# Avirup221/Multimodal-Hierarchical-CNN-for-Sun-Salutation-Pose-Classification

Measured on AMD Instinct MI355X. Metric: images/sec fwd+bwd QuadtreeCNN 224x224 bs256, higher is better.
Workload: dtype bf16; 1 GPU; QuadtreeCNN (ResNet-18 layer3, 2x2 split, 47-feat fusion) train step fwd+bwd+Adam, all parameters trainable; Adam(lr 1e-4, wd 1e-4) by the package's FusedAdam (csrc/pack.hip); global_batch=256, per_gpu_batch=256, image=3x224x224, num_classes=12, parallelism=dp1

## Files before the change

include/qtcnn.h:

```cpp
#ifndef QTCNN_H_
#define QTCNN_H_

#include <stddef.h>
#include <stdint.h>

#ifdef __cplusplus
extern "C" {
#endif

typedef enum qt_status {
  QT_OK = 0,
  QT_ERR_INVALID_ARG = -1,
  QT_ERR_LAUNCH = -2,
  QT_ERR_UNSUPPORTED = -3
} qt_status;

typedef enum qt_dtype { QT_F32 = 0, QT_BF16 = 1 } qt_dtype;

int qt_version(void);
const char* qt_last_error(void);

enum { QT_CONV_FWD = 0, QT_CONV_DGRAD = 1 };

typedef struct qt_conv_desc {
// ... 7 lines not shown
  int kh, kw, stride, pad;
  long long src_img_stride;
  int src_row_stride;
  int src_pix_stride;
  int quad;
  int relu;
  int dst_sub, dst_h, dst_w, dst_off_h, dst_off_w;
  int dst_merge;
  int dst_merge_res0;
  int kt, frames;
  int dst_merge_extra;
} qt_conv_desc;

typedef struct qt_conv_io {
  const void* src;
  const void* weight;
  void* dst;
  const float* scale;
  const float* shift;
  const void* residual;
  const void* relu_mask;
  float* stats_partial;
  struct {
    const void* y;
    const float* mean;
    const float* invstd;
    float* partial;
  } bwd_bn[2];
  const unsigned char* relu_mask_bits;
  const void* extra_src;
} qt_conv_io;

void qt_set_patch_conv(int mode);
void qt_set_pt_conv(int mode);
void qt_set_pt_conv_max_workgroups(int n);
void qt_set_stem_conv(int mode);
int qt_conv2d_stats_rows(const qt_conv_desc* desc);
typedef struct qt_conv_s2_desc {
  int dtype;
  int batch;
  int in_h, in_w;
  int c_in, c_out;
  int relu_conv, relu_down;
} qt_conv_s2_desc;
typedef struct qt_conv_s2_io {
  const void* src;
  const void* w_conv;
  const void* w_down;
  void* y_conv;
  void* y_down;
  const float* scale_conv;
  const float* shift_conv;
  const float* scale_down;
  const float* shift_down;
  float* stats_conv;
  float* stats_down;
} qt_conv_s2_io;
int qt_conv_s2_pair_supported(const qt_conv_s2_desc* desc);
int qt_conv_s2_pair_stats_rows(const qt_conv_s2_desc* desc);
int qt_conv_s2_pair(const qt_conv_s2_desc* desc, const qt_conv_s2_io* io, void* stream);
void qt_set_conv_s2(int mode);
void qt_set_conv_s2_max_workgroups(int n);

int qt_conv2d_igemm(const qt_conv_desc* desc, const qt_conv_io* io, void* stream);

int qt_conv2d_wgrad(const qt_conv_desc* desc, const void* dy, const void* x, float* dw, void* stream);
// ... 228 lines not shown
```

multimodal-hierarchical-cnn-for-sun-salutation-pose-classification_amd/csrc/conv_patch.hip:

```cpp
#include <stdlib.h>

#include <type_traits>

#include "qt_common.h"

namespace {

struct PatchArgs {
  const void* src;
  const void* wgt;
  void* dst;
  const float* scale;
  const float* shift;
  const void* residual;
  const void* relu_mask;
  const unsigned char* relu_mask_bits;
  float* stats_partial;
  const void* bn_y[2];
  const float* bn_mean[2];
  const float* bn_invstd[2];
  float* bn_partial[2];
  int B, H, W, C, N;
  int PW, PP;
  long long Q;
  int flip;
  int relu;
  int gridM, gridN;
  FastDiv div_pp, div_pw;
};

constexpr int kRowBytes = 128;
constexpr int BM = 256;
constexpr int NT = 512;

constexpr int L1_PW = 58, L1_RING = 640, L1_MIRROR = 48, L1_WBYTES = 9 * 64 * kRowBytes;
constexpr int L1_RBYTES = (L1_RING + L1_MIRROR) * kRowBytes;
constexpr int L1_RED = 0;
constexpr int L1_LDS = L1_WBYTES + L1_RBYTES;
static_assert(L1_LDS <= 160 * 1024 && 8 * 2 * 4 * 4 * 3 * 4 <= L1_WBYTES, "layer1 ring kernel LDS");

__device__ uint4 l1_store_sink[NT];

template <bool FLIP, bool OPS>
__global__ __launch_bounds__(NT) void conv_l1_ring_kernel(PatchArgs p) {
  using T = bf16_t;
  extern __shared__ __attribute__((aligned(16))) unsigned char smem[];
  const T* __restrict__ src = static_cast<const T*>(p.src);
  const T* __restrict__ wgt = static_cast<const T*>(p.wgt);
  const int tid = threadIdx.x, lane = tid & 63;
  const int wave = __builtin_amdgcn_readfirstlane(tid >> 6);
  const int wm = wave & 3, wn = wave >> 2;
  const int frow = lane & 15, fk = lane >> 4;
  const int rbase = tid >> 3, chunk = (tid & 7) ^ (rbase & 7);
  const unsigned smem_base = lds_addr_of(smem);
  const T* zero_src = reinterpret_cast<const T*>(qt_zero_page);

  const int ntiles = p.gridM, G = gridDim.x, b = blockIdx.x;
  const int t0 = (int)((long long)b * ntiles / G), t1 = (int)((long long)(b + 1) * ntiles / G);
  const int nt = t1 - t0;
  if (nt <= 0) return;
  const long long qstart = (long long)t0 * BM - (L1_PW + 1);

  auto dma_ring = [&](int ub) {
    const long long q = qstart + ub + rbase;
    const T* g = zero_src;
    if (q >= 0 && q < p.Q) {
      const unsigned uq = (unsigned)q;
      const unsigned img = fdiv(uq, p.div_pp);
      const unsigned rem = uq - img * (unsigned)p.PP;
      const unsigned hp = fdiv(rem, p.div_pw);
      const unsigned wp = rem - hp * (unsigned)L1_PW;
      if (hp >= 1 && hp <= 56u && wp >= 1 && wp <= 56u)
        g = src + (((long long)img * 56 + (hp - 1)) * 56 + (wp - 1)) * 64 + chunk * 8;
    }
    const int rrow = __builtin_amdgcn_readfirstlane(ub % L1_RING);
    glds16(g, smem_base + L1_WBYTES + (rrow + wave * 8) * kRowBytes);
    if (rrow == 0 && wave < L1_MIRROR / 8)
// ... 6 lines not shown
    const int x = rbase & 15, ii = (rbase >> 4) & 1;
    const int chan = (rbase & 32) + 8 * (x >> 2) + 4 * ii + (x & 3);
    glds16(wgt + ((long long)chan * 9 + t) * 64 + chunk * 8, smem_base + (t * 64 + wave * 8) * kRowBytes);
  }
#pragma unroll
  for (int i = 0; i < 6; ++i) dma_ring(i * 64);

  float sc[2][4], sh[2][4], mu0[2][4], is0[2][4], mu1[2][4], is1[2][4];
  const bool bwd_stats = p.bn_y[0] != nullptr;
#pragma unroll
  for (int i = 0; i < 2; ++i)
#pragma unroll
    for (int r = 0; r < 4; ++r) {
      const int n = wn * 32 + fk * 8 + i * 4 + r;
      sc[i][r] = p.scale ? p.scale[n] : 1.f;
      sh[i][r] = p.shift ? p.shift[n] : 0.f;
      mu0[i][r] = bwd_stats ? p.bn_mean[0][n] : 0.f;
      is0[i][r] = bwd_stats ? p.bn_invstd[0][n] : 0.f;
      mu1[i][r] = p.bn_y[1] ? p.bn_mean[1][n] : 0.f;
      is1[i][r] = p.bn_y[1] ? p.bn_invstd[1][n] : 0.f;
    }
  float s1[2][4], s2[2][4], s3[2][4];
#pragma unroll
  for (int i = 0; i < 2; ++i)
#pragma unroll
    for (int r = 0; r < 4; ++r) s1[i][r] = s2[i][r] = s3[i][r] = 0.f;
  T* __restrict__ dst = static_cast<T*>(p.dst);
  const T* __restrict__ res = static_cast<const T*>(p.residual);
  const T* __restrict__ msk = static_cast<const T*>(p.relu_mask);
  const unsigned char* __restrict__ mbits = p.relu_mask_bits;
  const unsigned char* ring = smem + L1_WBYTES;
  const int w_lane = (wn * 32 + frow) * kRowBytes + ((fk ^ (frow & 7)) << 4);

  int base = 0;
  for (int k = 0; k < nt; ++k) {
    if (k == 0)
      asm volatile("s_waitcnt vmcnt(0) lgkmcnt(0)\n\ts_barrier" ::: "memory");
    else
      asm volatile("s_waitcnt vmcnt(4) lgkmcnt(0)\n\ts_barrier" ::: "memory");
    if (k + 1 < nt) {
#pragma unroll
      for (int i = 0; i < 4; ++i) dma_ring(256 * k + 384 + i * 64);
    }
    auto out_row = [&](int j) -> int {
      const long long q = (long long)(t0 + k) * BM + wm * 64 + j * 16 + frow;
      if (q >= p.Q) return -1;
      const unsigned uq = (unsigned)q;
      const unsigned img = fdiv(uq, p.div_pp);
      const unsigned rem = uq - img * (unsigned)p.PP;
      const unsigned hp = fdiv(rem, p.div_pw);
      const unsigned wp = rem - hp * (unsigned)L1_PW;
      return (hp >= 1 && hp <= 56u && wp >= 1 && wp <= 56u) ? (int)((img * 56 + (hp - 1)) * 56 + (wp - 1)) : -1;
    };
    int prow[4] = {-1, -1, -1, -1};
    uint4 pre_res[4], pre_msk[4], pre_y0[4], pre_y1[4];
    if constexpr (OPS) {
#pragma unroll
      for (int j = 0; j < 4; ++j) {
        prow[j] = out_row(j);
        pre_res[j] = pre_msk[j] = pre_y0[j] = pre_y1[j] = make_uint4(0u, 0u, 0u, 0u);
        if (prow[j] >= 0) {
          const long long off = (long long)prow[j] * 64 + wn * 32 + fk * 8;
          if (res) pre_res[j] = *reinterpret_cast<const uint4*>(res + off);
          if (msk) pre_msk[j] = *reinterpret_cast<const uint4*>(msk + off);
          if (mbits) pre_msk[j].x = mbits[off >> 3];
          if (bwd_stats) pre_y0[j] = *reinterpret_cast<const uint4*>(static_cast<const T*>(p.bn_y[0]) + off);
          if (p.bn_y[1]) pre_y1[j] = *reinterpret_cast<const uint4*>(static_cast<const T*>(p.bn_y[1]) + off);
        }
      }
    }
    f32x4 acc[2][4];
#pragma unroll
    for (int i = 0; i < 2; ++i)
#pragma unroll
      for (int j = 0; j < 4; ++j) acc[i][j] = (f32x4){0.f, 0.f, 0.f, 0.f};
    const int lane_row = base + wm * 64 + frow;
    uint4 fwp[2][2], fap[2][4];
    auto read_group = [&](int g, uint4 (&fw)[2], uint4 (&fa)[4]) {
      constexpr int kPW = L1_PW;
      const int t = g >> 1, kk = g & 1;
      const int kh = t / 3, kw = t % 3;
      const int shift = FLIP ? (2 - kh) * kPW + (2 - kw) : kh * kPW + kw;
      int rr0 = lane_row + shift;
      rr0 = rr0 >= L1_RING ? rr0 - L1_RING : rr0;
      const int a0 = rr0 * kRowBytes + ((fk ^ ((frow + shift) & 7)) << 4);
#pragma unroll
      for (int i = 0; i < 2; ++i)
        fw[i] = *reinterpret_cast<const uint4*>(smem + (w_lane ^ (kk << 6)) + (t * 64 + i * 16) * kRowBytes);
#pragma unroll
      for (int j = 0; j < 4; ++j)
        fa[j] = *reinterpret_cast<const uint4*>(ring + (a0 ^ (kk << 6)) + j * (16 * kRowBytes));
    };
    read_group(0, fwp[0], fap[0]);
#pragma unroll
    for (int g = 0; g < 18; ++g) {
      if (g + 1 < 18) read_group(g + 1, fwp[(g + 1) & 1], fap[(g + 1) & 1]);
      __builtin_amdgcn_sched_barrier(0);
      __builtin_amdgcn_s_setprio(1);
#pragma unroll
      for (int i = 0; i < 2; ++i)
#pragma unroll
        for (int j = 0; j < 4; ++j) QtMma<T>::run(acc[i][j], fwp[g & 1][i], fap[g & 1][j]);
      __builtin_amdgcn_s_setprio(0);
      __builtin_amdgcn_sched_barrier(0);
    }
    base += BM;
    if (base >= L1_RING) base -= L1_RING;

    auto bf4 = [](unsigned lo, unsigned hi, float (&f)[4]) {
      f[0] = __uint_as_float(lo << 16); f[1] = __uint_as_float(lo & 0xffff0000u);
      f[2] = __uint_as_float(hi << 16); f[3] = __uint_as_float(hi & 0xffff0000u);
    };
#pragma unroll
    for (int j = 0; j < 4; ++j) {
      if constexpr (!OPS) prow[j] = out_row(j);
      const bool live = prow[j] >= 0;
      const float lm = live ? 1.f : 0.f;
      const long long off = (long long)(live ? prow[j] : 0) * 64 + wn * 32 + fk * 8;
      bf16x8 o;
#pragma unroll
      for (int i = 0; i < 2; ++i) {
        float v[4] = {acc[i][j][0], acc[i][j][1], acc[i][j][2], acc[i][j][3]};
        if (p.stats_partial != nullptr && !bwd_stats) {
#pragma unroll
          for (int r = 0; r < 4; ++r) {
// ... 69 lines not shown
        for (int r = 0; r < 4; ++r) {
          float* d = red + ((((wave * 2 + i) * 4 + fk) * 4 + r) * 3);
          d[0] = s1[i][r];
          d[1] = s2[i][r];
          d[2] = s3[i][r];
        }
    }
    __syncthreads();
    if (tid < 64) {
      const int n = tid, wn_ = n >> 5, fk_ = (n >> 3) & 3, i = (n >> 2) & 1, r = n & 3;
      float a = 0.f, bb = 0.f, c = 0.f;
      for (int w4 = 0; w4 < 4; ++w4) {
        const float* d = red + (((((wn_ * 4 + w4) * 2 + i) * 4 + fk_) * 4 + r) * 3);
        a += d[0];
        bb += d[1];
        c += d[2];
      }
      float* o0 = bwd_stats ? p.bn_partial[0] : p.stats_partial;
      o0[((long long)b * 2 + 0) * 64 + n] = a;
      o0[((long long)b * 2 + 1) * 64 + n] = bb;
      if (bwd_stats && p.bn_y[1]) {
        p.bn_partial[1][((long long)b * 2 + 0) * 64 + n] = a;
        p.bn_partial[1][((long long)b * 2 + 1) * 64 + n] = c;
      }
    }
  }
}

inline int l1_ring_grid(long long Q) {
  const int ntiles = qt_cdiv(Q, BM);
  return ntiles < 256 ? ntiles : 256;
}

template <bool FLIP, bool OPS>
int launch_l1_ring(PatchArgs a, hipStream_t stream) {
  auto kern = conv_l1_ring_kernel<FLIP, OPS>;
  static std::atomic<unsigned long long> lds_limit_set{0};
  if (int rc = qt_raise_lds_limit(reinterpret_cast<const void*>(kern), L1_LDS, lds_limit_set)) return rc;
  a.gridM = qt_cdiv(a.Q, BM);
  a.gridN = 1;
  hipLaunchKernelGGL(kern, dim3(l1_ring_grid(a.Q)), dim3(NT), L1_LDS, stream, a);
  QT_CHECK_LAUNCH();
  return QT_OK;
}

}



static int g_patch_enabled = -1;
extern "C" void qt_set_patch_conv(int mode) { g_patch_enabled = mode < 0 ? 2 : (mode > 2 ? 2 : mode); }

static bool l1_ring_shape(const qt_conv_desc* d);

bool qt_patch_eligible(const qt_conv_desc* d) {
  if (g_patch_enabled < 0) {
    const char* v = getenv("QTCNN_PATCH_CONV");
    g_patch_enabled = v ? atoi(v) : 2;
  }
  if (!g_patch_enabled) return false;
  return l1_ring_shape(d) && d->kh == 3 && d->kw == 3 && d->stride == 1 && d->pad == 1 && !d->quad && !d->dst_sub &&
         d->in_h == d->out_h && d->in_w == d->out_w && d->in_h == d->in_w && d->src_pix_stride == d->k_per_tap &&
         d->src_row_stride == d->in_w * d->k_per_tap &&
         d->src_img_stride == (long long)d->in_h * d->in_w * d->k_per_tap &&
         (long long)d->batch * (d->in_h + 2) * (d->in_w + 2) < (1ll << 31);
}

static bool l1_ring_shape(const qt_conv_desc* d) {
  return d->dtype == QT_BF16 && d->in_w == 56 && d->k_per_tap == 64 && d->n_out == 64;
}

int qt_patch_stats_rows(const qt_conv_desc* d) {
  const long long Q = (long long)d->batch * (d->in_h + 2) * (d->in_w + 2);
  return l1_ring_grid(Q);
}

int qt_patch_launch(const qt_conv_desc* d, const qt_conv_io* io, void* stream) {
  PatchArgs a;
  a.src = io->src; a.wgt = io->weight; a.dst = io->dst;
  a.scale = io->scale; a.shift = io->shift; a.residual = io->residual; a.relu_mask = io->relu_mask;
  a.relu_mask_bits = io->relu_mask_bits;
  a.stats_partial = io->stats_partial;
  for (int k = 0; k < 2; ++k) {
    a.bn_y[k] = io->bwd_bn[k].y; a.bn_mean[k] = io->bwd_bn[k].mean; a.bn_invstd[k] = io->bwd_bn[k].invstd;
    a.bn_partial[k] = io->bwd_bn[k].partial;
  }
  a.B = d->batch; a.H = d->in_h; a.W = d->in_w; a.C = d->k_per_tap; a.N = d->n_out;
  a.PW = a.W + 2; a.PP = (a.H + 2) * a.PW;
  a.Q = (long long)a.B * a.PP;
  a.flip = d->mode == QT_CONV_DGRAD;
  a.relu = d->relu;
  a.div_pp = make_fastdiv((unsigned)a.PP);
  a.div_pw = make_fastdiv((unsigned)a.PW);
  a.gridM = a.gridN = 0;
  hipStream_t s = static_cast<hipStream_t>(stream);
  const bool ops = a.residual || a.relu_mask || a.relu_mask_bits || a.bn_y[0];
  if (a.flip) return ops ? launch_l1_ring<true, true>(a, s) : launch_l1_ring<true, false>(a, s);
  return ops ? launch_l1_ring<false, true>(a, s) : launch_l1_ring<false, false>(a, s);
}
```

multimodal-hierarchical-cnn-for-sun-salutation-pose-classification_amd/csrc/conv_wgrad_s2.hip:

```cpp
#include <stdlib.h>

#include "qt_common.h"

int qt_wgrad_partial_sum_launch(const float* part, float* dw, size_t filt, int nsplit, int KC, int layout, hipStream_t stream);

namespace {

constexpr int T = 64;
constexpr int CH = 32;

struct WS2Args {
  const bf16_t* dy;
  const bf16_t* x;
  float* part;
  unsigned x_is2, dy_is2;
  int x_rs, x_ps;
  int N, KC, OH, OW, PW, PP, B;
  int total, pps, nsplit, tiles, tilesC;
  int HL;
  unsigned xrb, bufb, tab;
  unsigned x_bytes, dy_bytes;
  FastDiv div_pp, div_pw;
  int tap_plane[9], tap_shift[9];
};

__device__ __forceinline__ QT_LDS_AS s16x4* lds_tr_ptr(unsigned lds_byte) { return (QT_LDS_AS s16x4*)(size_t)lds_byte; }

template <int NPL, int NTAP, int NB, int NU>
__global__ __launch_bounds__(512) void conv_wgrad_s2_kernel(WS2Args a) {
  extern __shared__ __attribute__((aligned(16))) unsigned char smem[];
  if (lds_addr_of(smem) != 0) return;

  const int tid = threadIdx.x, lane = tid & 63;
  const int wave = __builtin_amdgcn_readfirstlane(tid >> 6);
  const int group = wave >> 2, wq = wave & 3;

  int split, tile;
  if ((a.nsplit & 7) == 0) {
    const int xcd = blockIdx.x & 7, slot = blockIdx.x >> 3;
    split = (slot / a.tiles) * 8 + xcd;
    tile = slot % a.tiles;
  } else {
    split = blockIdx.x % a.nsplit;
    tile = blockIdx.x / a.nsplit;
  }
  const int tc = tile % a.tilesC, tn = tile / a.tilesC;
  const int n0 = tn * 64, c0 = tc * 64;
  const int p0 = split * a.pps;
  if (p0 >= a.total) return;
  const int pend = min(a.total, p0 + a.pps);
  const int ntiles = (pend - p0 + T - 1) / T;

  const int tabn = a.PP + 8;
  {
    unsigned* tx = reinterpret_cast<unsigned*>(smem + a.tab);
    unsigned* ty = tx + tabn;
    for (int r = tid; r < tabn; r += 512) {
      const int rr = r >= a.PP ? r - a.PP : r;
      const int ph = (int)fdiv((unsigned)rr, a.div_pw), pw = rr - ph * a.PW;
      const bool ok = ph >= 1 && pw >= 1;
      const unsigned nx = r >= a.PP ? a.x_is2 : 0u, ny = r >= a.PP ? a.dy_is2 : 0u;
      tx[r] = ok ? (unsigned)(2 * (ph - 1) * a.x_rs + 2 * (pw - 1) * a.x_ps) * 2u + nx : kOob;
      ty[r] = ok ? (unsigned)(((ph - 1) * a.OW + (pw - 1)) * a.N) * 2u + ny : kOob;
    }
  }

  const i32x4 rx = make_rsrc(a.x, a.x_bytes), ry = make_rsrc(a.dy, a.dy_bytes);
  const int drow = lane >> 3, dslot = lane & 7;
  const int dkey = (drow >> 1) & 3;
  const unsigned lane_c = (unsigned)((((dslot >> 1) ^ dkey) << 1) | (dslot & 1)) * 16u;
  const unsigned tab_x = a.tab + (unsigned)drow * 4u, tab_y = tab_x + (unsigned)tabn * 4u;
  const int xu = (T + a.HL) >> 3;
  const int xunits = NPL * xu;
  auto sgpr = [](unsigned v) -> unsigned { return (unsigned)__builtin_amdgcn_readfirstlane((int)v); };
  auto split_pos = [&](int pos, unsigned& img1, unsigned& rem) {
    const unsigned g = (unsigned)(pos + a.PP);
    img1 = fdiv(g, a.div_pp);
    rem = g - img1 * (unsigned)a.PP;
  };
  const unsigned spare = a.tab + 2u * (unsigned)tabn * 4u;
  auto dma_tile = [&](int k, unsigned bufbase) {
    const int q0 = p0 + k * T;
#pragma unroll
    for (int j = 0; j < NU - 1; ++j) {
      const int u = wave + 8 * j;
      const bool live = u < xunits;
      const int uc = live ? u : 0;
      const int pl = NPL == 1 ? 0 : uc / xu, uu = NPL == 1 ? uc : uc - pl * xu;
      unsigned img1, rem;
      split_pos(q0 - a.HL + 8 * uu, img1, rem);
      const unsigned plane_off = (unsigned)((pl >> 1) * a.x_rs + (pl & 1) * a.x_ps) * 2u;
      const unsigned base = sgpr((img1 - 1u) * a.x_is2 + (unsigned)c0 * 2u + plane_off);
      const unsigned tv = *reinterpret_cast<const unsigned*>(smem + tab_x + sgpr(rem) * 4u);
      i32x4 r_ = rx;
      r_.z = (int)sgpr(live ? a.x_bytes : 0u);
      blds16(r_, tv + base + lane_c, 0u, sgpr(live ? bufbase + (unsigned)pl * a.xrb + (unsigned)uu * 1024u : spare));
    }
    {
      unsigned img1, rem;
      split_pos(q0 + 8 * wave, img1, rem);
      const unsigned base = sgpr((img1 - 1u) * a.dy_is2 + (unsigned)n0 * 2u);
      const unsigned tv = *reinterpret_cast<const unsigned*>(smem + tab_y + sgpr(rem) * 4u);
      blds16(ry, tv + base + lane_c, 0u, sgpr(bufbase + (unsigned)NPL * a.xrb + (unsigned)wave * 1024u));
    }
  };

  const int li = lane & 15, lg = lane >> 4;
  const int qq = li >> 2, pp = li & 3;
  const int lrow = 4 * lg + qq;
  unsigned a_base[4], b_base[NTAP];
#pragma unroll
  for (int i = 0; i < 4; ++i)
    a_base[i] = (unsigned)NPL * a.xrb + (unsigned)(group * CH + lrow) * 128u + ((unsigned)(i ^ ((lrow >> 1) & 3)) << 5) + pp * 8;
#pragma unroll
  for (int t = 0; t < NTAP; ++t) {
    const int r = a.HL + a.tap_shift[t] + group * CH + lrow;
    b_base[t] = (unsigned)a.tap_plane[t] * a.xrb + (unsigned)r * 128u + ((unsigned)(wq ^ ((r >> 1) & 3)) << 5) + pp * 8;
  }
  auto frag = [&](unsigned addr) -> uint4 {
    s16x4 lo = __builtin_amdgcn_ds_read_tr16_b64_v4i16(lds_tr_ptr(addr));
    s16x4 hi = __builtin_amdgcn_ds_read_tr16_b64_v4i16(lds_tr_ptr(addr + 2048));
    uint2 l2 = __builtin_bit_cast(uint2, lo), h2 = __builtin_bit_cast(uint2, hi);
    return make_uint4(l2.x, l2.y, h2.x, h2.y);
  };

  f32x4 acc[4][NTAP];
#pragma unroll
  for (int i = 0; i < 4; ++i)
#pragma unroll
    for (int t = 0; t < NTAP; ++t) acc[i][t] = (f32x4){0.f, 0.f, 0.f, 0.f};

  asm volatile("s_waitcnt lgkmcnt(0)\n\ts_barrier" ::: "memory");
#pragma unroll
  for (int t = 0; t < NB - 1; ++t) dma_tile(t, (unsigned)t * a.bufb);
  asm volatile("s_waitcnt vmcnt(%0) lgkmcnt(0)\n\ts_barrier" ::"n"(NU * (NB - 2)) : "memory");

  unsigned wbuf = (unsigned)(NB - 1) * a.bufb;
  int rbuf = 0;
  for (int k = 0; k < ntiles; ++k) {
    dma_tile(k + NB - 1, wbuf);
    wbuf = wbuf + a.bufb == (unsigned)NB * a.bufb ? 0u : wbuf + a.bufb;
    uint4 fa[4], fb[3];
#pragma unroll
    for (int i = 0; i < 4; ++i) fa[i] = frag(a_base[i]);
    fb[0] = frag(b_base[0]);
    if (NTAP > 1) fb[1] = frag(b_base[NTAP > 1 ? 1 : 0]);
#pragma unroll
    for (int t = 0; t < NTAP; ++t) {
      if (t + 2 < NTAP) fb[(t + 2) % 3] = frag(b_base[t + 2 < NTAP ? t + 2 : 0]);
      __builtin_amdgcn_s_setprio(1);
#pragma unroll
      for (int i = 0; i < 4; ++i)
        acc[i][t] = __builtin_amdgcn_mfma_f32_16x16x32_bf16(__builtin_bit_cast(bf16x8, fa[i]),
                                                            __builtin_bit_cast(bf16x8, fb[t % 3]), acc[i][t], 0, 0, 0);
      __builtin_amdgcn_s_setprio(0);
    }
    {
      rbuf = rbuf + 1 == NB ? 0 : rbuf + 1;
      const unsigned delta = rbuf == 0 ? 0u - (unsigned)(NB - 1) * a.bufb : a.bufb;
#pragma unroll
      for (int i = 0; i < 4; ++i) {
        a_base[i] += delta;
        asm volatile("" : "+v"(a_base[i]));
      }
#pragma unroll
      for (int t = 0; t < NTAP; ++t) {
        b_base[t] += delta;
        asm volatile("" : "+v"(b_base[t]));
      }
    }
    asm volatile("s_waitcnt vmcnt(%0) lgkmcnt(0)\n\ts_barrier" ::"n"(NU * (NB - 2)) : "memory");
  }
  asm volatile("s_waitcnt vmcnt(0)" ::: "memory");
  __syncthreads();

  {
    f32x4* xch = reinterpret_cast<f32x4*>(smem) + (wq * 2 * NTAP) * 64 + lane;
    if (group == 1) {
#pragma unroll
      for (int i = 0; i < 2; ++i)
#pragma unroll
        for (int t = 0; t < NTAP; ++t) xch[(i * NTAP + t) * 64] = acc[i][t];
    }
    __syncthreads();
    if (group == 0) {
#pragma unroll
      for (int i = 0; i < 2; ++i)
#pragma unroll
        for (int t = 0; t < NTAP; ++t) acc[i][t] += xch[(i * NTAP + t) * 64];
    }
    __syncthreads();
    if (group == 0) {
#pragma unroll
      for (int i = 0; i < 2; ++i)
#pragma unroll
        for (int t = 0; t < NTAP; ++t) xch[(i * NTAP + t) * 64] = acc[2 + i][t];
    }
    __syncthreads();
    if (group == 1) {
#pragma unroll
      for (int i = 0; i < 2; ++i)
// ... 33 lines not shown

int s2_buffers() {
  static int v = -1;
  if (v < 0) {
    const char* e = getenv("QTCNN_S2_BUFFERS");
    v = e ? atoi(e) : 3;
  }
  return v;
}

void split_ranges(int total, int tiles, int* pps_out, int* nsplit_out) {
  int nsplit = 256 / tiles;
  if (nsplit < 1) nsplit = 1;
  int pps = qt_cdiv(total, nsplit);
  pps = qt_cdiv(pps, T) * T;
  *pps_out = pps;
  *nsplit_out = qt_cdiv(total, pps);
}

}

extern "C" void qt_set_wgrad_s2(int on) { g_wgrad_s2 = on < 0 ? 1 : on; }

bool qt_wgrad_s2_eligible(const qt_conv_desc* d) {
  if (!s2_enabled() || d->dtype != QT_BF16 || d->stride != 2 || d->quad || d->kt > 1) return false;
  const bool k3 = d->kh == 3 && d->kw == 3 && d->pad == 1, k1 = d->kh == 1 && d->kw == 1 && d->pad == 0;
  if (!k3 && !k1) return false;
  if ((d->in_h & 1) || (d->in_w & 1) || d->out_h * 2 != d->in_h || d->out_w * 2 != d->in_w) return false;
  if (d->n_out % 64 || d->k_per_tap % 64) return false;
  if (d->out_w < 4 || d->out_w > 120 || d->out_h < 4) return false;
  if ((long long)d->batch * d->src_img_stride * 2 >= (1ll << 30)) return false;
  if ((long long)d->batch * d->out_h * d->out_w * d->n_out * 2 >= (1ll << 30)) return false;
  if ((long long)d->batch * (d->out_h + 1) * (d->out_w + 1) >= (1ll << 30)) return false;
  const int PW = d->out_w + 1, HL = (PW + 1 + 7) / 8 * 8;
  const unsigned npl = k3 ? 4u : 1u;
  const unsigned lds = 2u * ((npl * (unsigned)(T + HL) + (unsigned)T) * 128u) + 2u * (unsigned)((d->out_h + 1) * PW + 8) * 4u + 1024u;
  const int nu = qt_cdiv((int)npl * ((T + HL) / 8), 8) + 1;
  if (k3 ? (nu != 6 && nu != 7) : (nu != 2 && nu != 3)) return false;
  return lds <= 160u * 1024u && HL <= (d->out_h + 1) * PW;
}

size_t qt_wgrad_s2_workspace_bytes(const qt_conv_desc* d) {
  if (!qt_wgrad_s2_eligible(d)) return 0;
  const int total = d->batch * (d->out_h + 1) * (d->out_w + 1);
  int pps, nsplit;
  split_ranges(total, (d->n_out / 64) * (d->k_per_tap / 64), &pps, &nsplit);
  return (size_t)nsplit * d->n_out * d->kh * d->kw * d->k_per_tap * 4;
}

int qt_wgrad_s2_launch(const qt_conv_desc* d, const void* dy, const void* x, float* grad_oihw, void* workspace,
                       size_t workspace_bytes, void* stream) {
  const bool k3 = d->kh == 3;
  WS2Args a;
  a.dy = static_cast<const bf16_t*>(dy);
  a.x = static_cast<const bf16_t*>(x);
  a.part = static_cast<float*>(workspace);
  a.N = d->n_out; a.KC = d->k_per_tap; a.OH = d->out_h; a.OW = d->out_w; a.B = d->batch;
  a.PW = a.OW + 1; a.PP = a.PW * (a.OH + 1);
  a.x_rs = d->src_row_stride; a.x_ps = d->src_pix_stride;
  a.x_is2 = (unsigned)(d->src_img_stride * 2);
  a.dy_is2 = (unsigned)((long long)a.OH * a.OW * a.N * 2);
  a.x_bytes = (unsigned)((long long)a.B * d->src_img_stride * 2);
  a.dy_bytes = (unsigned)((long long)a.B * a.OH * a.OW * a.N * 2);
  a.total = a.B * a.PP;
  a.HL = (a.PW + 1 + 7) / 8 * 8;
  a.div_pp = make_fastdiv((unsigned)a.PP);
  a.div_pw = make_fastdiv((unsigned)a.PW);
  a.tilesC = a.KC / 64;
  a.tiles = (a.N / 64) * a.tilesC;
  int real_split;
  split_ranges(a.total, a.tiles, &a.pps, &real_split);
  a.nsplit = real_split;
  if (a.nsplit >= 6 && (a.nsplit & 7)) a.nsplit = qt_cdiv(a.nsplit, 8) * 8;
  const int ntap = k3 ? 9 : 1, npl = k3 ? 4 : 1;
  const size_t filt = (size_t)a.N * ntap * a.KC;
  if (!workspace || workspace_bytes < (size_t)real_split * filt * 4) {
    qt_set_error("qt_conv2d_wgrad_oihw: workspace of %zu bytes needed", (size_t)real_split * filt * 4);
    return QT_ERR_INVALID_ARG;
  }
  a.xrb = (unsigned)(T + a.HL) * 128u;
  a.bufb = (unsigned)npl * a.xrb + (unsigned)T * 128u;
  const unsigned tab_bytes = 2u * (unsigned)(a.PP + 8) * 4u + 1024u;
  const int nb = (3u * a.bufb + tab_bytes <= 160u * 1024u && s2_buffers() >= 3) ? 3 : 2;
  a.tab = (unsigned)nb * a.bufb;
  const int nu = qt_cdiv(npl * ((T + a.HL) / 8), 8) + 1;
  for (int t = 0; t < 9; ++t) {
    const int kh = k3 ? t / 3 : 1, kw = k3 ? t % 3 : 1;
    a.tap_plane[t] = k3 ? ((kh != 1) * 2 + (kw != 1)) : 0;
    a.tap_shift[t] = -((kh == 0) * a.PW + (kw == 0));
  }
  const unsigned lds = a.tab + tab_bytes;
  if ((size_t)2 * a.bufb < (size_t)4 * 2 * ntap * 64 * 16) {
    qt_set_error("qt_conv2d_wgrad_oihw: map too small for the stride-2 kernel");
    return QT_ERR_UNSUPPORTED;
  }
  hipStream_t s = static_cast<hipStream_t>(stream);
#define QT_S2_LAUNCH(NPL_, NTAP_, NB_, NU_)                                                                     \
  {                                                                                                             \
    auto kern = conv_wgrad_s2_kernel<NPL_, NTAP_, NB_, NU_>;                                                    \
    static std::atomic<unsigned long long> set_{0};                                                             \
    if (int rc = qt_raise_lds_limit(reinterpret_cast<const void*>(kern), 160 * 1024, set_)) return rc;          \
    hipLaunchKernelGGL(kern, dim3(a.tiles * a.nsplit), dim3(512), lds, s, a);                                   \
    launched = true;                                                                                            \
  }
  bool launched = false;
  if (k3 && nb == 3 && nu == 6) QT_S2_LAUNCH(4, 9, 3, 6)
  else if (k3 && nb == 3 && nu == 7) QT_S2_LAUNCH(4, 9, 3, 7)
  else if (k3 && nu == 6) QT_S2_LAUNCH(4, 9, 2, 6)
  else if (k3 && nu == 7) QT_S2_LAUNCH(4, 9, 2, 7)
  else if (!k3 && nb == 3 && nu == 3) QT_S2_LAUNCH(1, 1, 3, 3)
  else if (!k3 && nb == 3 && nu == 2) QT_S2_LAUNCH(1, 1, 3, 2)
  else if (!k3 && nu == 3) QT_S2_LAUNCH(1, 1, 2, 3)
  else if (!k3 && nu == 2) QT_S2_LAUNCH(1, 1, 2, 2)
#undef QT_S2_LAUNCH
  if (!launched) {
    qt_set_error("qt_conv2d_wgrad_oihw: stride-2 kernel: no instantiation for this map width");
    return QT_ERR_UNSUPPORTED;
  }
  QT_CHECK_LAUNCH();
  return qt_wgrad_partial_sum_launch(a.part, grad_oihw, filt, real_split, a.KC, k3 ? 1 : 2, s);
}
```

Before: 46020 images/s.

## Overlap layer1 ring conv epilogue with next tile's MFMA loop

Adds a pipelined variant of the layer1 ring conv kernel for the no-memory-operand case. It double-buffers the accumulators, and the previous tile's epilogue (address calc, stats accumulation, affine/relu, bf16 pack, global store) is interleaved into the next tile's 18 MFMA groups using sched_group_barrier hints. The ring DMA prefetches are also spread across the first groups instead of issued up front. This aims to hide epilogue latency behind matrix work, at the cost of doubled accumulator registers and a spill risk. It is enabled by default and can be turned off with QTCNN_L1_PIPE=0.

```diff
diff --git a/include/qtcnn.h b/include/qtcnn.h
--- a/include/qtcnn.h
+++ b/include/qtcnn.h
@@ -63,6 +63,7 @@
 } qt_conv_io;
 
 void qt_set_patch_conv(int mode);
+void qt_set_l1_pipe(int mode);
 void qt_set_pt_conv(int mode);
 void qt_set_pt_conv_max_workgroups(int n);
 void qt_set_stem_conv(int mode);
diff --git a/multimodal-hierarchical-cnn-for-sun-salutation-pose-classification_amd/csrc/conv_patch.hip b/multimodal-hierarchical-cnn-for-sun-salutation-pose-classification_amd/csrc/conv_patch.hip
--- a/multimodal-hierarchical-cnn-for-sun-salutation-pose-classification_amd/csrc/conv_patch.hip
+++ b/multimodal-hierarchical-cnn-for-sun-salutation-pose-classification_amd/csrc/conv_patch.hip
@@ -41,8 +41,9 @@
 
 __device__ uint4 l1_store_sink[NT];
 
-template <bool FLIP, bool OPS>
+template <bool FLIP, bool OPS, int PIPE>
 __global__ __launch_bounds__(NT) void conv_l1_ring_kernel(PatchArgs p) {
+  static_assert(PIPE == 0 || !OPS, "the pipelined epilogue has no memory operands");
   using T = bf16_t;
   extern __shared__ __attribute__((aligned(16))) unsigned char smem[];
   const T* __restrict__ src = static_cast<const T*>(p.src);
@@ -115,7 +116,154 @@
   const unsigned char* ring = smem + L1_WBYTES;
   const int w_lane = (wn * 32 + frow) * kRowBytes + ((fk ^ (frow & 7)) << 4);
 
+  auto read_group_at = [&](int lane_row, int g, uint4 (&fw)[2], uint4 (&fa)[4]) {
+    constexpr int kPW = L1_PW;
+    const int t = g >> 1, kk = g & 1;
+    const int kh = t / 3, kw = t % 3;
+    const int shift = FLIP ? (2 - kh) * kPW + (2 - kw) : kh * kPW + kw;
+    int rr0 = lane_row + shift;
+    rr0 = rr0 >= L1_RING ? rr0 - L1_RING : rr0;
+    const int a0 = rr0 * kRowBytes + ((fk ^ ((frow + shift) & 7)) << 4);
+#pragma unroll
+    for (int i = 0; i < 2; ++i)
+      fw[i] = *reinterpret_cast<const uint4*>(smem + (w_lane ^ (kk << 6)) + (t * 64 + i * 16) * kRowBytes);
+#pragma unroll
+    for (int j = 0; j < 4; ++j)
+      fa[j] = *reinterpret_cast<const uint4*>(ring + (a0 ^ (kk << 6)) + j * (16 * kRowBytes));
+  };
+  auto out_row_at = [&](int tile, int j) -> int {
+    const long long q = (long long)tile * BM + wm * 64 + j * 16 + frow;
+    if (q >= p.Q) return -1;
+    const unsigned uq = (unsigned)q;
+    const unsigned img = fdiv(uq, p.div_pp);
+    const unsigned rem = uq - img * (unsigned)p.PP;
+    const unsigned hp = fdiv(rem, p.div_pw);
+    const unsigned wp = rem - hp * (unsigned)L1_PW;
+    return (hp >= 1 && hp <= 56u && wp >= 1 && wp <= 56u) ? (int)((img * 56 + (hp - 1)) * 56 + (wp - 1)) : -1;
+  };
+
   int base = 0;
+  if constexpr (PIPE != 0) {
+    if constexpr (PIPE == 2) {
+#pragma unroll
+      for (int i = 0; i < 2; ++i)
+#pragma unroll
+        for (int r = 0; r < 4; ++r) asm volatile("" ::"v"(sc[i][r]), "v"(sh[i][r]));
+    }
+    float lm = 0.f;
+    bf16x8* outp = nullptr;
+    bf16x8 o;
+    auto part_addr = [&](int tile, int j) {
+      int fr = frow;
+      asm volatile("" : "+v"(fr));
+      const long long q = (long long)tile * BM + wm * 64 + j * 16 + fr;
+      const unsigned uq = (unsigned)q;
+      const unsigned img = fdiv(uq, p.div_pp);
+      const unsigned rem = uq - img * (unsigned)p.PP;
+      const unsigned hp = fdiv(rem, p.div_pw);
+      const unsigned wp = rem - hp * (unsigned)L1_PW;
+      const bool live = q < p.Q && hp >= 1 && hp <= 56u && wp >= 1 && wp <= 56u;
+      const int row = (int)((img * 56 + (hp - 1)) * 56 + (wp - 1));
+      lm = live ? 1.f : 0.f;
+      const long long off = (long long)(live ? row : 0) * 64 + wn * 32 + fk * 8;
+      outp = live ? reinterpret_cast<bf16x8*>(dst + off) : reinterpret_cast<bf16x8*>(&l1_store_sink[tid]);
+      asm volatile("" ::"v"(lm), "v"(outp));
+    };
+    auto part_half = [&](const f32x4 (&prv)[2][4], int j, int i) {
+      float v[4] = {prv[i][j][0], prv[i][j][1], prv[i][j][2], prv[i][j][3]};
+      asm volatile("" : "+v"(v[0]), "+v"(v[1]), "+v"(v[2]), "+v"(v[3]));
+#pragma unroll
+      for (int r = 0; r < 4; ++r) {
+        s1[i][r] += lm * v[r];
+        s2[i][r] += lm * v[r] * v[r];
+      }
+      if constexpr (PIPE == 2) {
+        const bool affine = p.scale || p.shift, relu = p.relu;
+#pragma unroll
+        for (int r = 0; r < 4; ++r) v[r] = affine ? v[r] * sc[i][r] + sh[i][r] : v[r];
+#pragma unroll
+        for (int r = 0; r < 4; ++r) v[r] = relu ? fmaxf(v[r], 0.f) : v[r];
+      }
+#pragma unroll
+      for (int r = 0; r < 4; ++r) o[i * 4 + r] = (bf16_t)v[r];
+      asm volatile("" ::"v"(o), "v"(s1[i][0]), "v"(s1[i][1]), "v"(s1[i][2]), "v"(s1[i][3]), "v"(s2[i][0]), "v"(s2[i][1]),
+                   "v"(s2[i][2]), "v"(s2[i][3]));
+    };
+    auto part_store = [&]() {
+      asm volatile("global_store_dwordx4 %0, %1, off\n\ts_nop 1" ::"v"(outp), "v"(o) : "memory");
+    };
+    auto epilogue = [&](const f32x4 (&prv)[2][4], int tile) {
+#pragma unroll
+      for (int j = 0; j < 4; ++j) {
+        part_addr(tile, j);
+        part_half(prv, j, 0);
+        part_half(prv, j, 1);
+        part_store();
+      }
+    };
+    auto tile_step = [&](int k, f32x4 (&acc)[2][4], const f32x4 (&prv)[2][4], auto has_prev) {
+      constexpr bool HAS_PREV = decltype(has_prev)::value;
+      if (k < 2)
+        asm volatile("s_waitcnt vmcnt(0) lgkmcnt(0)\n\ts_barrier" ::: "memory");
+      else
+        asm volatile("s_waitcnt vmcnt(4) lgkmcnt(0)\n\ts_barrier" ::: "memory");
+      const bool fetch = k + 1 < nt;
+#pragma unroll
+      for (int i = 0; i < 2; ++i)
+#pragma unroll
+        for (int j = 0; j < 4; ++j) acc[i][j] = (f32x4){0.f, 0.f, 0.f, 0.f};
+      const int lane_row = base + wm * 64 + frow;
+      uint4 fwp[2][2], fap[2][4];
+      read_group_at(lane_row, 0, fwp[0], fap[0]);
+#pragma unroll
+      for (int g = 0; g < 18; ++g) {
+        if (g + 1 < 18) read_group_at(lane_row, g + 1, fwp[(g + 1) & 1], fap[(g + 1) & 1]);
+        if (g < 4 && fetch) dma_ring(256 * k + 384 + g * 64);
+        __builtin_amdgcn_sched_barrier(0);
+        __builtin_amdgcn_s_setprio(1);
+#pragma unroll
+        for (int i = 0; i < 2; ++i)
+#pragma unroll
+          for (int j = 0; j < 4; ++j) QtMma<T>::run(acc[i][j], fwp[g & 1][i], fap[g & 1][j]);
+        bool store = false;
+        if constexpr (HAS_PREV) {
+#pragma unroll
+          for (int m = 0; m < 12; ++m) {
+            if ((3 * m) / 2 != g) continue;
+            const int j = m / 3;
+            if (m % 3 == 0) part_addr(t0 + k - 1, j);
+            else part_half(prv, j, m % 3 - 1);
+            store = store || m % 3 == 2;
+#pragma unroll
+            for (int s = 0; s < 8; ++s) {
+              __builtin_amdgcn_sched_group_barrier(0x008, 1, 0);
+              __builtin_amdgcn_sched_group_barrier(0x002, 3, 0);
+            }
+          }
+        }
+        __builtin_amdgcn_s_setprio(0);
+        __builtin_amdgcn_sched_barrier(0);
+        if (store) part_store();
+      }
+      base += BM;
+      if (base >= L1_RING) base -= L1_RING;
+    };
+    using NoPrev = std::integral_constant<bool, false>;
+    using Prev = std::integral_constant<bool, true>;
+    f32x4 accA[2][4], accB[2][4];
+    tile_step(0, accA, accB, NoPrev{});
+    int k = 1;
+    for (; k + 1 < nt; k += 2) {
+      tile_step(k, accB, accA, Prev{});
+      tile_step(k + 1, accA, accB, Prev{});
+    }
+    if (k < nt) {
+      tile_step(k, accB, accA, Prev{});
+      epilogue(accB, t0 + k);
+    } else {
+      epilogue(accA, t0 + k - 1);
+    }
+  } else
   for (int k = 0; k < nt; ++k) {
     if (k == 0)
       asm volatile("s_waitcnt vmcnt(0) lgkmcnt(0)\n\ts_barrier" ::: "memory");
@@ -125,16 +273,7 @@
 #pragma unroll
       for (int i = 0; i < 4; ++i) dma_ring(256 * k + 384 + i * 64);
     }
-    auto out_row = [&](int j) -> int {
-      const long long q = (long long)(t0 + k) * BM + wm * 64 + j * 16 + frow;
-      if (q >= p.Q) return -1;
-      const unsigned uq = (unsigned)q;
-      const unsigned img = fdiv(uq, p.div_pp);
-      const unsigned rem = uq - img * (unsigned)p.PP;
-      const unsigned hp = fdiv(rem, p.div_pw);
-      const unsigned wp = rem - hp * (unsigned)L1_PW;
-      return (hp >= 1 && hp <= 56u && wp >= 1 && wp <= 56u) ? (int)((img * 56 + (hp - 1)) * 56 + (wp - 1)) : -1;
-    };
+    auto out_row = [&](int j) -> int { return out_row_at(t0 + k, j); };
     int prow[4] = {-1, -1, -1, -1};
     uint4 pre_res[4], pre_msk[4], pre_y0[4], pre_y1[4];
     if constexpr (OPS) {
@@ -159,21 +298,7 @@
       for (int j = 0; j < 4; ++j) acc[i][j] = (f32x4){0.f, 0.f, 0.f, 0.f};
     const int lane_row = base + wm * 64 + frow;
     uint4 fwp[2][2], fap[2][4];
-    auto read_group = [&](int g, uint4 (&fw)[2], uint4 (&fa)[4]) {
-      constexpr int kPW = L1_PW;
-      const int t = g >> 1, kk = g & 1;
-      const int kh = t / 3, kw = t % 3;
-      const int shift = FLIP ? (2 - kh) * kPW + (2 - kw) : kh * kPW + kw;
-      int rr0 = lane_row + shift;
-      rr0 = rr0 >= L1_RING ? rr0 - L1_RING : rr0;
-      const int a0 = rr0 * kRowBytes + ((fk ^ ((frow + shift) & 7)) << 4);
-#pragma unroll
-      for (int i = 0; i < 2; ++i)
-        fw[i] = *reinterpret_cast<const uint4*>(smem + (w_lane ^ (kk << 6)) + (t * 64 + i * 16) * kRowBytes);
-#pragma unroll
-      for (int j = 0; j < 4; ++j)
-        fa[j] = *reinterpret_cast<const uint4*>(ring + (a0 ^ (kk << 6)) + j * (16 * kRowBytes));
-    };
+    auto read_group = [&](int g, uint4 (&fw)[2], uint4 (&fa)[4]) { read_group_at(lane_row, g, fw, fa); };
     read_group(0, fwp[0], fap[0]);
 #pragma unroll
     for (int g = 0; g < 18; ++g) {
@@ -309,9 +434,9 @@
   return ntiles < 256 ? ntiles : 256;
 }
 
-template <bool FLIP, bool OPS>
+template <bool FLIP, bool OPS, int PIPE = 0>
 int launch_l1_ring(PatchArgs a, hipStream_t stream) {
-  auto kern = conv_l1_ring_kernel<FLIP, OPS>;
+  auto kern = conv_l1_ring_kernel<FLIP, OPS, PIPE>;
   static std::atomic<unsigned long long> lds_limit_set{0};
   if (int rc = qt_raise_lds_limit(reinterpret_cast<const void*>(kern), L1_LDS, lds_limit_set)) return rc;
   a.gridM = qt_cdiv(a.Q, BM);
@@ -327,6 +452,9 @@
 
 static int g_patch_enabled = -1;
 extern "C" void qt_set_patch_conv(int mode) { g_patch_enabled = mode < 0 ? 2 : (mode > 2 ? 2 : mode); }
+
+static int g_l1_pipe = -1;
+extern "C" void qt_set_l1_pipe(int mode) { g_l1_pipe = mode < 0 ? -1 : (mode ? 1 : 0); }
 
 static bool l1_ring_shape(const qt_conv_desc* d);
 
@@ -372,6 +500,13 @@
   a.gridM = a.gridN = 0;
   hipStream_t s = static_cast<hipStream_t>(stream);
   const bool ops = a.residual || a.relu_mask || a.relu_mask_bits || a.bn_y[0];
-  if (a.flip) return ops ? launch_l1_ring<true, true>(a, s) : launch_l1_ring<true, false>(a, s);
-  return ops ? launch_l1_ring<false, true>(a, s) : launch_l1_ring<false, false>(a, s);
-}
+  if (ops) return a.flip ? launch_l1_ring<true, true>(a, s) : launch_l1_ring<false, true>(a, s);
+  if (g_l1_pipe < 0) {
+    const char* v = getenv("QTCNN_L1_PIPE");
+    g_l1_pipe = v ? (atoi(v) ? 1 : 0) : 1;
+  }
+  if (!g_l1_pipe) return a.flip ? launch_l1_ring<true, false>(a, s) : launch_l1_ring<false, false>(a, s);
+  if (a.scale || a.shift || a.relu)
+    return a.flip ? launch_l1_ring<true, false, 2>(a, s) : launch_l1_ring<false, false, 2>(a, s);
+  return a.flip ? launch_l1_ring<true, false, 1>(a, s) : launch_l1_ring<false, false, 1>(a, s);
+}
```

After: 46280 images/s (median of 6 runs). About the same (+0.6%).

## Use ring buffer for stride-2 wgrad input planes to stop reloading halo rows

Applied to the files above, without the earlier changes.

Replaces the per-stage input buffers of the stride-2 weight-gradient kernel, each of which held a full halo plus tile, with a circular ring of rows per plane. The halo is loaded once in the prologue and each pipeline step then fetches only the new tile rows. This is meant to cut redundant global-to-LDS traffic and the DMA instruction count, and it makes the halo width a template parameter. In exchange, B-fragment addresses need wraparound logic every iteration, eligibility is narrowed to small map widths, and the budget used to pick three buffers is tightened.

```diff
diff --git a/multimodal-hierarchical-cnn-for-sun-salutation-pose-classification_amd/csrc/conv_wgrad_s2.hip b/multimodal-hierarchical-cnn-for-sun-salutation-pose-classification_amd/csrc/conv_wgrad_s2.hip
--- a/multimodal-hierarchical-cnn-for-sun-salutation-pose-classification_amd/csrc/conv_wgrad_s2.hip
+++ b/multimodal-hierarchical-cnn-for-sun-salutation-pose-classification_amd/csrc/conv_wgrad_s2.hip
@@ -17,17 +17,26 @@
   int x_rs, x_ps;
   int N, KC, OH, OW, PW, PP, B;
   int total, pps, nsplit, tiles, tilesC;
-  int HL;
-  unsigned xrb, bufb, tab;
+  unsigned tab;
   unsigned x_bytes, dy_bytes;
   FastDiv div_pp, div_pw;
-  int tap_plane[9], tap_shift[9];
+  int tap_shift[9];
 };
 
+__host__ __device__ constexpr unsigned s2_ring_rows(int nb, int hl) { return (unsigned)(nb * T + hl); }
+__host__ __device__ constexpr unsigned s2_ring_bytes(int npl, int nb, int hl) {
+  return (unsigned)npl * s2_ring_rows(nb, hl) * 128u + (unsigned)(nb * T) * 128u;
+}
+__host__ __device__ constexpr int s2_tap_plane(int ntap, int t) { return ntap == 1 ? 0 : ((t / 3 != 1) << 1) | (t % 3 != 1); }
+
 __device__ __forceinline__ QT_LDS_AS s16x4* lds_tr_ptr(unsigned lds_byte) { return (QT_LDS_AS s16x4*)(size_t)lds_byte; }
 
-template <int NPL, int NTAP, int NB, int NU>
+template <int NPL, int NTAP, int NB, int HL>
 __global__ __launch_bounds__(512) void conv_wgrad_s2_kernel(WS2Args a) {
+  static_assert((NPL * HL) % 64 == 0, "halo units: a whole number per wave");
+  constexpr unsigned R = s2_ring_rows(NB, HL), RB = R * 128u;
+  constexpr unsigned Y0 = (unsigned)NPL * RB, YB = T * 128u;
+  constexpr int NU = NPL + 1;
   extern __shared__ __attribute__((aligned(16))) unsigned char smem[];
   if (lds_addr_of(smem) != 0) return;
 
@@ -70,57 +79,44 @@
   const int dkey = (drow >> 1) & 3;
   const unsigned lane_c = (unsigned)((((dslot >> 1) ^ dkey) << 1) | (dslot & 1)) * 16u;
   const unsigned tab_x = a.tab + (unsigned)drow * 4u, tab_y = tab_x + (unsigned)tabn * 4u;
-  const int xu = (T + a.HL) >> 3;
-  const int xunits = NPL * xu;
   auto sgpr = [](unsigned v) -> unsigned { return (unsigned)__builtin_amdgcn_readfirstlane((int)v); };
   auto split_pos = [&](int pos, unsigned& img1, unsigned& rem) {
     const unsigned g = (unsigned)(pos + a.PP);
     img1 = fdiv(g, a.div_pp);
     rem = g - img1 * (unsigned)a.PP;
   };
-  const unsigned spare = a.tab + 2u * (unsigned)tabn * 4u;
-  auto dma_tile = [&](int k, unsigned bufbase) {
-    const int q0 = p0 + k * T;
-#pragma unroll
-    for (int j = 0; j < NU - 1; ++j) {
-      const int u = wave + 8 * j;
-      const bool live = u < xunits;
-      const int uc = live ? u : 0;
-      const int pl = NPL == 1 ? 0 : uc / xu, uu = NPL == 1 ? uc : uc - pl * xu;
-      unsigned img1, rem;
-      split_pos(q0 - a.HL + 8 * uu, img1, rem);
-      const unsigned plane_off = (unsigned)((pl >> 1) * a.x_rs + (pl & 1) * a.x_ps) * 2u;
-      const unsigned base = sgpr((img1 - 1u) * a.x_is2 + (unsigned)c0 * 2u + plane_off);
-      const unsigned tv = *reinterpret_cast<const unsigned*>(smem + tab_x + sgpr(rem) * 4u);
-      i32x4 r_ = rx;
-      r_.z = (int)sgpr(live ? a.x_bytes : 0u);
-      blds16(r_, tv + base + lane_c, 0u, sgpr(live ? bufbase + (unsigned)pl * a.xrb + (unsigned)uu * 1024u : spare));
-    }
-    {
-      unsigned img1, rem;
-      split_pos(q0 + 8 * wave, img1, rem);
-      const unsigned base = sgpr((img1 - 1u) * a.dy_is2 + (unsigned)n0 * 2u);
-      const unsigned tv = *reinterpret_cast<const unsigned*>(smem + tab_y + sgpr(rem) * 4u);
-      blds16(ry, tv + base + lane_c, 0u, sgpr(bufbase + (unsigned)NPL * a.xrb + (unsigned)wave * 1024u));
-    }
+  auto plane_off = [&](int pl) -> unsigned { return (unsigned)((pl >> 1) * a.x_rs + (pl & 1) * a.x_ps) * 2u; };
+  auto dma_tile = [&](int k) {
+    unsigned img1, rem;
+    split_pos(p0 + k * T + 8 * wave, img1, rem);
+    const unsigned xbase = (img1 - 1u) * a.x_is2 + (unsigned)c0 * 2u;
+    const unsigned tvx = *reinterpret_cast<const unsigned*>(smem + tab_x + sgpr(rem) * 4u) + lane_c;
+    const unsigned row = (unsigned)(HL + k * T + 8 * wave) % R;
+#pragma unroll
+    for (int pl = 0; pl < NPL; ++pl)
+      blds16(rx, tvx + sgpr(xbase + plane_off(pl)), 0u, sgpr((unsigned)pl * RB + row * 128u));
+    const unsigned ybase = sgpr((img1 - 1u) * a.dy_is2 + (unsigned)n0 * 2u);
+    const unsigned tvy = *reinterpret_cast<const unsigned*>(smem + tab_y + sgpr(rem) * 4u);
+    blds16(ry, tvy + ybase + lane_c, 0u, sgpr(Y0 + (unsigned)(k % NB) * YB + (unsigned)wave * 1024u));
   };
 
   const int li = lane & 15, lg = lane >> 4;
   const int qq = li >> 2, pp = li & 3;
   const int lrow = 4 * lg + qq;
-  unsigned a_base[4], b_base[NTAP];
+  unsigned a_base[4], b_lo[NTAP], b_hi[NTAP];
 #pragma unroll
   for (int i = 0; i < 4; ++i)
-    a_base[i] = (unsigned)NPL * a.xrb + (unsigned)(group * CH + lrow) * 128u + ((unsigned)(i ^ ((lrow >> 1) & 3)) << 5) + pp * 8;
+    a_base[i] = Y0 + (unsigned)(group * CH + lrow) * 128u + ((unsigned)(i ^ ((lrow >> 1) & 3)) << 5) + pp * 8;
 #pragma unroll
   for (int t = 0; t < NTAP; ++t) {
-    const int r = a.HL + a.tap_shift[t] + group * CH + lrow;
-    b_base[t] = (unsigned)a.tap_plane[t] * a.xrb + (unsigned)r * 128u + ((unsigned)(wq ^ ((r >> 1) & 3)) << 5) + pp * 8;
-  }
-  auto frag = [&](unsigned addr) -> uint4 {
-    s16x4 lo = __builtin_amdgcn_ds_read_tr16_b64_v4i16(lds_tr_ptr(addr));
-    s16x4 hi = __builtin_amdgcn_ds_read_tr16_b64_v4i16(lds_tr_ptr(addr + 2048));
-    uint2 l2 = __builtin_bit_cast(uint2, lo), h2 = __builtin_bit_cast(uint2, hi);
+    const int r = HL + a.tap_shift[t] + group * CH + lrow;
+    b_lo[t] = (unsigned)s2_tap_plane(NTAP, t) * RB + (unsigned)r * 128u + ((unsigned)(wq ^ ((r >> 1) & 3)) << 5) + pp * 8;
+    b_hi[t] = b_lo[t] + 2048u;
+  }
+  auto frag = [&](unsigned lo, unsigned hi) -> uint4 {
+    s16x4 l = __builtin_amdgcn_ds_read_tr16_b64_v4i16(lds_tr_ptr(lo));
+    s16x4 h = __builtin_amdgcn_ds_read_tr16_b64_v4i16(lds_tr_ptr(hi));
+    uint2 l2 = __builtin_bit_cast(uint2, l), h2 = __builtin_bit_cast(uint2, h);
     return make_uint4(l2.x, l2.y, h2.x, h2.y);
   };
 
@@ -132,22 +128,30 @@
 
   asm volatile("s_waitcnt lgkmcnt(0)\n\ts_barrier" ::: "memory");
 #pragma unroll
-  for (int t = 0; t < NB - 1; ++t) dma_tile(t, (unsigned)t * a.bufb);
+  for (int j = 0; j < NPL * HL / 64; ++j) {
+    constexpr int HPL = HL > 0 ? HL / 8 : 1;
+    const int h = wave + 8 * j, pl = h / HPL, uu = h - pl * HPL;
+    unsigned img1, rem;
+    split_pos(p0 - HL + 8 * uu, img1, rem);
+    const unsigned tv = *reinterpret_cast<const unsigned*>(smem + tab_x + sgpr(rem) * 4u);
+    blds16(rx, tv + sgpr((img1 - 1u) * a.x_is2 + (unsigned)c0 * 2u + plane_off(pl)) + lane_c, 0u,
+           sgpr((unsigned)pl * RB + (unsigned)uu * 1024u));
+  }
+#pragma unroll
+  for (int t = 0; t < NB - 1; ++t) dma_tile(t);
   asm volatile("s_waitcnt vmcnt(%0) lgkmcnt(0)\n\ts_barrier" ::"n"(NU * (NB - 2)) : "memory");
 
-  unsigned wbuf = (unsigned)(NB - 1) * a.bufb;
   int rbuf = 0;
   for (int k = 0; k < ntiles; ++k) {
-    dma_tile(k + NB - 1, wbuf);
-    wbuf = wbuf + a.bufb == (unsigned)NB * a.bufb ? 0u : wbuf + a.bufb;
+    dma_tile(k + NB - 1);
     uint4 fa[4], fb[3];
 #pragma unroll
-    for (int i = 0; i < 4; ++i) fa[i] = frag(a_base[i]);
-    fb[0] = frag(b_base[0]);
-    if (NTAP > 1) fb[1] = frag(b_base[NTAP > 1 ? 1 : 0]);
+    for (int i = 0; i < 4; ++i) fa[i] = frag(a_base[i], a_base[i] + 2048u);
+    fb[0] = frag(b_lo[0], b_hi[0]);
+    if (NTAP > 1) fb[1] = frag(b_lo[NTAP > 1 ? 1 : 0], b_hi[NTAP > 1 ? 1 : 0]);
 #pragma unroll
     for (int t = 0; t < NTAP; ++t) {
-      if (t + 2 < NTAP) fb[(t + 2) % 3] = frag(b_base[t + 2 < NTAP ? t + 2 : 0]);
+      if (t + 2 < NTAP) fb[(t + 2) % 3] = frag(b_lo[t + 2 < NTAP ? t + 2 : 0], b_hi[t + 2 < NTAP ? t + 2 : 0]);
       __builtin_amdgcn_s_setprio(1);
 #pragma unroll
       for (int i = 0; i < 4; ++i)
@@ -157,7 +161,7 @@
     }
     {
       rbuf = rbuf + 1 == NB ? 0 : rbuf + 1;
-      const unsigned delta = rbuf == 0 ? 0u - (unsigned)(NB - 1) * a.bufb : a.bufb;
+      const unsigned delta = rbuf == 0 ? 0u - (unsigned)(NB - 1) * YB : YB;
 #pragma unroll
       for (int i = 0; i < 4; ++i) {
         a_base[i] += delta;
@@ -165,8 +169,13 @@
       }
 #pragma unroll
       for (int t = 0; t < NTAP; ++t) {
-        b_base[t] += delta;
-        asm volatile("" : "+v"(b_base[t]));
+        constexpr unsigned step = T * 128u;
+        const unsigned end = (unsigned)(s2_tap_plane(NTAP, t) + 1) * RB;
+        b_lo[t] += step;
+        b_lo[t] = b_lo[t] >= end ? b_lo[t] - RB : b_lo[t];
+        b_hi[t] += step;
+        b_hi[t] = b_hi[t] >= end ? b_hi[t] - RB : b_hi[t];
+        asm volatile("" : "+v"(b_lo[t]), "+v"(b_hi[t]));
       }
     }
     asm volatile("s_waitcnt vmcnt(%0) lgkmcnt(0)\n\ts_barrier" ::"n"(NU * (NB - 2)) : "memory");
@@ -266,12 +275,11 @@
   if ((long long)d->batch * d->src_img_stride * 2 >= (1ll << 30)) return false;
   if ((long long)d->batch * d->out_h * d->out_w * d->n_out * 2 >= (1ll << 30)) return false;
   if ((long long)d->batch * (d->out_h + 1) * (d->out_w + 1) >= (1ll << 30)) return false;
-  const int PW = d->out_w + 1, HL = (PW + 1 + 7) / 8 * 8;
-  const unsigned npl = k3 ? 4u : 1u;
-  const unsigned lds = 2u * ((npl * (unsigned)(T + HL) + (unsigned)T) * 128u) + 2u * (unsigned)((d->out_h + 1) * PW + 8) * 4u + 1024u;
-  const int nu = qt_cdiv((int)npl * ((T + HL) / 8), 8) + 1;
-  if (k3 ? (nu != 6 && nu != 7) : (nu != 2 && nu != 3)) return false;
-  return lds <= 160u * 1024u && HL <= (d->out_h + 1) * PW;
+  const int PW = d->out_w + 1, PP = (d->out_h + 1) * PW;
+  if (PW + 1 > (k3 ? 32 : 64)) return false;
+  const int HL = k3 ? (PW + 1 + 15) / 16 * 16 : 0;
+  const unsigned lds = s2_ring_bytes(k3 ? 4 : 1, 2, HL) + 2u * (unsigned)(PP + 8) * 4u;
+  return lds <= 160u * 1024u && HL <= PP;
 }
 
 size_t qt_wgrad_s2_workspace_bytes(const qt_conv_desc* d) {
@@ -297,7 +305,7 @@
   a.x_bytes = (unsigned)((long long)a.B * d->src_img_stride * 2);
   a.dy_bytes = (unsigned)((long long)a.B * a.OH * a.OW * a.N * 2);
   a.total = a.B * a.PP;
-  a.HL = (a.PW + 1 + 7) / 8 * 8;
+  const int HL = k3 ? (a.PW + 1 + 15) / 16 * 16 : 0;
   a.div_pp = make_fastdiv((unsigned)a.PP);
   a.div_pw = make_fastdiv((unsigned)a.PW);
   a.tilesC = a.KC / 64;
@@ -312,40 +320,33 @@
     qt_set_error("qt_conv2d_wgrad_oihw: workspace of %zu bytes needed", (size_t)real_split * filt * 4);
     return QT_ERR_INVALID_ARG;
   }
-  a.xrb = (unsigned)(T + a.HL) * 128u;
-  a.bufb = (unsigned)npl * a.xrb + (unsigned)T * 128u;
-  const unsigned tab_bytes = 2u * (unsigned)(a.PP + 8) * 4u + 1024u;
-  const int nb = (3u * a.bufb + tab_bytes <= 160u * 1024u && s2_buffers() >= 3) ? 3 : 2;
-  a.tab = (unsigned)nb * a.bufb;
-  const int nu = qt_cdiv(npl * ((T + a.HL) / 8), 8) + 1;
+  const unsigned tab_bytes = 2u * (unsigned)(a.PP + 8) * 4u;
+  const int nb = (s2_ring_bytes(npl, 3, HL) + tab_bytes <= 136u * 1024u && s2_buffers() >= 3) ? 3 : 2;
+  a.tab = s2_ring_bytes(npl, nb, HL);
   for (int t = 0; t < 9; ++t) {
     const int kh = k3 ? t / 3 : 1, kw = k3 ? t % 3 : 1;
-    a.tap_plane[t] = k3 ? ((kh != 1) * 2 + (kw != 1)) : 0;
     a.tap_shift[t] = -((kh == 0) * a.PW + (kw == 0));
   }
   const unsigned lds = a.tab + tab_bytes;
-  if ((size_t)2 * a.bufb < (size_t)4 * 2 * ntap * 64 * 16) {
+  if ((size_t)a.tab < (size_t)4 * 2 * ntap * 64 * 16) {
     qt_set_error("qt_conv2d_wgrad_oihw: map too small for the stride-2 kernel");
     return QT_ERR_UNSUPPORTED;
   }
   hipStream_t s = static_cast<hipStream_t>(stream);
-#define QT_S2_LAUNCH(NPL_, NTAP_, NB_, NU_)                                                                     \
+#define QT_S2_LAUNCH(NPL_, NTAP_, NB_, HL_)                                                                     \
   {                                                                                                             \
-    auto kern = conv_wgrad_s2_kernel<NPL_, NTAP_, NB_, NU_>;                                                    \
+    auto kern = conv_wgrad_s2_kernel<NPL_, NTAP_, NB_, HL_>;                                                    \
     static std::atomic<unsigned long long> set_{0};                                                             \
     if (int rc = qt_raise_lds_limit(reinterpret_cast<const void*>(kern), 160 * 1024, set_)) return rc;          \
     hipLaunchKernelGGL(kern, dim3(a.tiles * a.nsplit), dim3(512), lds, s, a);                                   \
     launched = true;                                                                                            \
   }
   bool launched = false;
-  if (k3 && nb == 3 && nu == 6) QT_S2_LAUNCH(4, 9, 3, 6)
-  else if (k3 && nb == 3 && nu == 7) QT_S2_LAUNCH(4, 9, 3, 7)
-  else if (k3 && nu == 6) QT_S2_LAUNCH(4, 9, 2, 6)
-  else if (k3 && nu == 7) QT_S2_LAUNCH(4, 9, 2, 7)
-  else if (!k3 && nb == 3 && nu == 3) QT_S2_LAUNCH(1, 1, 3, 3)
-  else if (!k3 && nb == 3 && nu == 2) QT_S2_LAUNCH(1, 1, 3, 2)
-  else if (!k3 && nu == 3) QT_S2_LAUNCH(1, 1, 2, 3)
-  else if (!k3 && nu == 2) QT_S2_LAUNCH(1, 1, 2, 2)
+  if (k3 && nb == 3 && HL == 16) QT_S2_LAUNCH(4, 9, 3, 16)
+  else if (k3 && HL == 16) QT_S2_LAUNCH(4, 9, 2, 16)
+  else if (k3 && HL == 32) QT_S2_LAUNCH(4, 9, 2, 32)
+  else if (!k3 && nb == 3) QT_S2_LAUNCH(1, 1, 3, 0)
+  else if (!k3) QT_S2_LAUNCH(1, 1, 2, 0)
 #undef QT_S2_LAUNCH
   if (!launched) {
     qt_set_error("qt_conv2d_wgrad_oihw: stride-2 kernel: no instantiation for this map width");
```

After: 46380 images/s before, 46500 images/s after (median of 6 runs). About the same (+0.3%).
